# Zhen-Dong/CoDeNet

Hardware: AMD Instinct MI355X
Metric: images/sec CoDeNet1x 512x512 ctdet inference (deform hot path: deconv_layers; whole network in `e2e`) (higher is better)
Workload: dtype f32+i8 (W4A8: fp32 scale / gather, int8-MFMA pointwise on 8-bit activation and 4-bit weight codes, i32 sums); 1 GPU; CoDeNet1x config-c 512x512 W4A8, batch 64 per GPU, 3 deform stages (scale 1x1 -> QuantAct -> bilinear-gather depthwise 3x3 -> QuantAct -> pointwise 1x1 + folded BN -> ReLU -> QuantAct range; output channels-last at stage resolution for the native heads), running QuantAct ranges (reference-faithful), fused per-stage schedule, HIP-graph replay; preset=cfg3, global_batch=64

## Files before the change

### codenet_amd/_native.py

```python
import ctypes
import os
import subprocess

_HERE = os.path.dirname(os.path.abspath(__file__))
SO_PATH = os.path.join(_HERE, "lib", "libcodenet_dcn.so")
CSRC = os.path.join(_HERE, "csrc")

CDN_F32, CDN_F64, CDN_F16 = 0, 1, 2
_lib = None

_vp, _i, _i64, _f, _d = ctypes.c_void_p, ctypes.c_int, ctypes.c_int64, ctypes.c_float, ctypes.c_double

_SIGNATURES = {
    "cdn_abi_version": (ctypes.c_int, []),
    "cdn_last_error": (ctypes.c_char_p, []),
    "cdn_deform_conv_forward": (_i, [_vp] * 4 + [_i] + [_i64] * 5 + [_i] * 10 + [_vp]),
    "cdn_deform_conv_forward_scratch_bytes": (ctypes.c_size_t, [_i64] * 5 + [_i] * 10),
    "cdn_deform_conv_forward_scratch": (_i, [_vp] * 4 + [_i] + [_i64] * 5 + [_i] * 10 + [_vp, ctypes.c_size_t, _vp]),
    "cdn_deform_conv_backward_input": (_i, [_vp] * 6 + [_i] + [_i64] * 5 + [_i] * 10 + [_vp]),
    "cdn_deform_conv_backward_input_scratch_bytes": (ctypes.c_size_t, [_i64] * 5 + [_i] * 10),
    "cdn_deform_conv_backward_input_scratch_min_bytes": (ctypes.c_size_t, [_i64] * 5 + [_i] * 10),
    "cdn_deform_conv_backward_input_scratch": (_i, [_vp] * 6 + [_i] + [_i64] * 5 + [_i] * 10 + [_vp, ctypes.c_size_t, _vp]),
    "cdn_deform_conv_backward_parameters": (_i, [_vp] * 4 + [_i] + [_i64] * 5 + [_i] * 10 + [_f, _vp]),
    "cdn_modulated_deform_conv_forward": (_i, [_vp] * 6 + [_i] + [_i64] * 5 + [_i] * 11 + [_vp]),
    "cdn_modulated_deform_conv_backward": (_i, [_vp] * 11 + [_i] + [_i64] * 5 + [_i] * 11 + [_vp]),
    "cdn_codenet_scale_forward": (_i, [_vp] * 4 + [_i64] * 4 + [_f, _f, _vp]),
    "cdn_codenet_dw_forward": (_i, [_vp] * 4 + [_i64] * 4 + [_vp]),
    "cdn_codenet_dw_backward_supported": (_i, [_i64, _i64]),
    "cdn_codenet_pointwise_wgrad_workspace_bytes": (ctypes.c_size_t, [_i64] * 4),
    "cdn_codenet_pointwise_wgrad": (_i, [_vp] * 4 + [_i64] * 4 + [_vp, ctypes.c_size_t, _vp]),
    "cdn_codenet_scale_backward": (_i, [_vp] * 5 + [_i64] * 4 + [_vp]),
    "cdn_codenet_scale_range_partials": (_i64, [_i64] * 3),
    "cdn_codenet_scale_forward_range": (_i, [_vp] * 4 + [_i64] * 4 + [_f, _f, _vp, _vp]),
    "cdn_codenet_dw_range_partials": (_i64, [_i64] * 4),
    "cdn_codenet_dw_forward_range": (_i, [_vp] * 4 + [_i64] * 4 + [_vp, _vp]),
    "cdn_codenet_pointwise_range_partials": (_i64, [_i64] * 3),
    "cdn_codenet_pointwise_forward_range": (_i, [_vp] * 7 + [_i64] * 4 + [_i, _vp, _vp]),
    "cdn_quantact_forward_partials": (_i, [_vp, _vp, _i64, _vp, _vp, _vp, _vp, _i64, _i, _d, _i, _vp, _vp]),
    "cdn_codenet_pointwise_wgrad_q": (_i, [_vp] * 5 + [_i64] * 4 + [_vp, ctypes.c_size_t, _vp]),
    "cdn_codenet_pointwise_wgrad_q_f32": (_i, [_vp] * 5 + [_i64] * 4 + [_vp, ctypes.c_size_t, _vp]),
    "cdn_quantact_relu_up2_forward_partials": (
        _i, [_vp, _vp] + [_i64] * 3 + [_vp] * 4 + [_i64, _i, _d, _i, _vp]),
    "cdn_codenet_scale_backward_masked": (_i, [_vp] * 3 + [_f, _f] + [_vp] * 3 + [_i64] * 4 + [_vp]),
    "cdn_codenet_weight_prep_backward": (_i, [_vp] * 7 + [_i64, _i64] + [_vp] * 5),
    "cdn_codenet_weight_prep": (_i, [_vp, _i64, _i64] + [_vp] * 4 + [_i] + [_vp] * 3),
    "cdn_codenet_weight_prep_multi": (_i, [_i] + [_vp] * 14),
    "cdn_codenet_weight_prep_ranked": (_i, [_vp, _i64, _i64] + [_vp] * 4 + [_i, _i, _i, _f] + [_vp] * 3),
    "cdn_codenet_stage_supported": (_i, [_i64] * 4 + [_i, _i]),
    "cdn_codenet_stage_fused_supported": (_i, [_i64] * 4 + [_i, _i]),
    "cdn_codenet_stage_chain_parts": (_i, [_i64] * 5),
    "cdn_codenet_heads_pointwise_supported": (_i, [_i64, _i64, _i]),
    "cdn_codenet_heads_pointwise_forward": (_i, [_vp, _vp, _i64, _i64, _i] + [_vp] * 5 + [_i] + [_vp] * 3 + [_i, _d, _i]
                                            + [_vp, ctypes.c_size_t, _vp, _vp, _i64, _vp]),
    "cdn_codenet_stage_fused_forward_chain": (_i, [_vp, _i, _i, _vp] + [_i64] * 5 + [_vp, _vp, _f, _f] + [_vp] * 5
                                              + [_i, _vp, ctypes.c_size_t, _vp, _vp, _i, _vp, _vp, _vp]),
    "cdn_codenet_stage_fused_intermediates": (_i, [_i64] * 4 + [_i, _i, _i, _vp, _vp]),
    "cdn_codenet_wcodes_kb_columns": (_i64, [_i64, _i64]),
    "cdn_codenet_pointwise_i8_supported": (_i, [_i64] * 4),
    "cdn_quantact_arrive_words": (_i, []),
    "cdn_codenet_scale_forward_update": (_i, [_vp] * 4 + [_i64] * 4 + [_f, _f] + [_vp] * 4 + [_i, _d, _vp, _vp]),
    "cdn_codenet_dw_forward_update_supported": (_i, [_i64] * 4 + [_i]),
    "cdn_codenet_dw_forward_update": (_i, [_vp] * 4 + [_i64] * 4 + [_i] + [_vp] * 4 + [_i, _d, _vp, _vp]),
    "cdn_codenet_pointwise_i8_forward_update": (_i, [_vp] * 5 + [_i64] * 4 + [_vp, ctypes.c_size_t, _i] + [_vp] * 4
                                                + [_i, _d, _vp]),
    "cdn_quantact_apply": (_i, [_vp, _vp, _i64, _vp, _vp]),
    "cdn_quantact_relu_apply": (_i, [_vp, _vp, _i64, _i64, _i64, _i, _vp, _vp]),
    "cdn_codenet_pointwise_dgrad_q4_supported": (_i, [_i64] * 4),
    "cdn_codenet_pointwise_dgrad_q4": (_i, [_vp] * 3 + [_i64] * 4 + [_vp]),
    "cdn_codenet_pointwise_i8_workspace_bytes": (ctypes.c_size_t, [_i64] * 4),
    "cdn_codenet_pointwise_i8_range_partials": (_i64, [_i64] * 4),
    "cdn_codenet_pointwise_i8_forward_range": (_i, [_vp] * 5 + [_i64] * 4 + [_vp, _vp, ctypes.c_size_t, _vp]),
    "cdn_codenet_wcodes_kb_offset": (_i64, [_i64, _i64]),
    "cdn_codenet_maxpool3x3s2_q8_forward": (_i, [_vp] + [_i64] * 6 + [_vp, _vp]),
    "cdn_codenet_dwpw_q8_supported": (_i, [_i64] * 3 + [_i, _i64]),
    "cdn_codenet_dwpw_q8_forward": (
        _i, [_vp, _vp] + [_i64] * 4 + [_i, _i64, _vp, _vp, _i, _vp, _i64] + [_vp] * 4 + [_i, _i64] + [_vp] * 5),
    "cdn_codenet_dw_backward": (_i, [_vp] * 7 + [_i64] * 4 + [_vp]),
    "cdn_codenet_dw_backward_workspace_bytes": (ctypes.c_size_t, [_i64] * 4 + [_i]),
    "cdn_codenet_dw_backward_r": (_i, [_vp] * 7 + [_i64] * 4 + [_vp, _vp]),
    "cdn_codenet_dw_up2_backward_r": (_i, [_vp] * 7 + [_i64] * 4 + [_vp, _vp]),
    "cdn_codenet_pointwise_forward": (_i, [_vp] * 6 + [_i64] * 4 + [_i, _vp]),
    "cdn_quantact_state_bytes": (ctypes.c_size_t, []),
    "cdn_kth_values_workspace_bytes": (ctypes.c_size_t, []),
    "cdn_kth_values": (_i, [_vp, _i64, _i64, _i64, _vp, _vp, _vp, ctypes.c_size_t, _vp]),
    "cdn_quantact_forward": (_i, [_vp] * 3 + [_i64] + [_vp] * 5 + [_i, _d, _i, _vp]),
    "cdn_quantact_relu_up2_forward": (_i, [_vp, _vp] + [_i64] * 3 + [_vp] * 3 + [_i, _d, _i, _vp]),
    "cdn_up2_relu_backward": (_i, [_vp] * 3 + [_i64] * 3 + [_vp]),
    "cdn_quantact_relu_forward": (_i, [_vp, _vp, _i64] + [_vp] * 4 + [_i64, _i, _d, _i, _vp]),
    "cdn_relu_backward": (_i, [_vp] * 3 + [_i64, _vp]),
    "cdn_codenet_pwdw_s2_supported": (_i, [_i64] * 5),
    "cdn_codenet_pwdw_s2_forward": (
        _i, [_vp, _vp] + [_i64] * 5 + [_vp] * 8 + [_i64, _vp, _vp, _i64] + [_vp] * 3 + [_i, _d, _i, _vp,
                                                                                    ctypes.c_size_t, _vp, _vp]),
    "cdn_codenet_pwdw_s2_apply": (
        _i, [_vp, _vp] + [_i64] * 5 + [_vp] * 8 + [_i64, _vp, _vp, _i64] + [_vp] * 3 + [_i, _d, _i, _vp,
                                                                                    ctypes.c_size_t, _vp, _vp]),
    "cdn_codenet_dw_up2_supported": (_i, [_i64] * 4),
    "cdn_codenet_dw_up2_range_partials": (_i64, [_i64] * 4),
    "cdn_codenet_dw_up2_forward": (_i, [_vp] * 4 + [_i64] * 4 + [_vp, _vp]),
    "cdn_codenet_dw_up2_backward": (_i, [_vp] * 7 + [_i64] * 4 + [_vp]),
    "cdn_codenet_stage_workspace_bytes": (ctypes.c_size_t, [_i64] * 4 + [_i]),
    "cdn_codenet_stage_fused_forward": (
        _i, [_vp, _i, _i, _vp] + [_i64] * 5 + [_vp, _vp, _f, _f] + [_vp] * 8 + [_i] + [_vp] * 9
        + [_i, _d, _i, _vp, ctypes.c_size_t, _vp, _vp]),
    "cdn_quantact_commit_range": (_i, [_vp, _vp, _vp, _vp, _i, _d, _i, _vp]),
    "cdn_quantact_frozen_params": (_i, [_i, _vp, _vp, _vp, _i, _vp]),
    "cdn_quantact_frozen_params_clear": (_i, [_i, _vp, _vp, _vp, _i, _vp, ctypes.c_size_t, _vp]),
    "cdn_codenet_stage_frozen_workspace_bytes": (ctypes.c_size_t, [_i64] * 4 + [_i]),
    "cdn_codenet_stage_frozen_forward": (
        _i, [_vp, _i, _i, _vp] + [_i64] * 5 + [_vp, _vp, _f, _f] + [_vp] * 5 + [_i] + [_vp] * 4
# ... 161 lines not shown
```

### codenet_amd/csrc/codenet_pointwise.hip

```cpp
#include "cdn_common.h"

#include <algorithm>
#include <type_traits>

#ifdef CDN_STAMPS
__device__ unsigned long long cdn_pw_stamps[2048 * 8];
#define CDN_STAMPR(R, I)                                                                              \
  do {                                                                                                \
    static_assert((R) == 2, "the pointwise kernels stamp region 2");                                  \
    if (threadIdx.x == 0)                                                                             \
      cdn_pw_stamps[((blockIdx.y * gridDim.x + blockIdx.x) & 2047) * 8 + (I)] = __builtin_amdgcn_s_memrealtime(); \
  } while (0)
int cdn::read_pointwise_stamps(unsigned long long *host_dst) {
  return (int)hipMemcpyFromSymbol(host_dst, HIP_SYMBOL(cdn_pw_stamps), sizeof(unsigned long long) * 2048 * 8);
}
int cdn::clear_pointwise_stamps() {
  void *p = nullptr;
  if (hipGetSymbolAddress(&p, HIP_SYMBOL(cdn_pw_stamps)) != hipSuccess) return 1;
  return (int)hipMemset(p, 0, sizeof(unsigned long long) * 2048 * 8);
}
#else
#define CDN_STAMPR(R, I) do { } while (0)
#endif

// ... 676 lines not shown
          if (relu) v = cdn::relu_keep_nan(v);
          if (R) R[m * ldo + oc] = v;
          mn = fminf(mn, v);
          mx = fmaxf(mx, v);
          has_nan |= (v != v);
        }
      }
  }
  CDN_STAMPR(2, 3);
  if (qu.tracks())
    cdn::block_minmax_finish(cdn::nan_lo(mn, has_nan), cdn::nan_hi(mx, has_nan), pidx, npart, qu,
                             reinterpret_cast<float *>(&A0[0][0]));
  CDN_STAMPR(2, 4);
}

template <int BM, int BN, int WGM, bool FAST>
__global__ void __launch_bounds__(256)
pwi8_kernel(const float *__restrict__ A, const unsigned *__restrict__ aq,
            const signed char *__restrict__ Wq, const float *__restrict__ wscale,
            const int *__restrict__ wsum, const float *__restrict__ Wp,
            const float *__restrict__ bias, float *__restrict__ R,
            cdn::QUpdate qu, long M, int C, int Cpad, int Co, int relu, int lda,
            int ldo, const int *__restrict__ omap, int Cw) {
  pwi8_body<BM, BN, WGM, FAST>(A, aq, Wq, wscale, wsum, Wp, bias, R, qu, M, C, Cpad, Co, relu, lda, ldo, omap, Cw,
                               (long)blockIdx.x * BM, blockIdx.y * BN, blockIdx.y * gridDim.x + blockIdx.x,
                               gridDim.x * gridDim.y);
}

struct QUpdateN {
  cdn::QUpdate q[4];
};
template <int NH>
__global__ void __launch_bounds__(256)
pwi8h_kernel(const float *__restrict__ A, const unsigned *__restrict__ aq, const signed char *__restrict__ Wq,
             const float *__restrict__ wscale, const int *__restrict__ wsum, const float *__restrict__ Wp,
             const float *__restrict__ bias, float *__restrict__ R, QUpdateN qus, long M, int C, int Cpad,
             int relu, int lda, const int *__restrict__ omap, long head_stride) {
  const int ntm = (int)((M + 63) / 64), grp = 8 * NH, b = blockIdx.x, full = (ntm / 8) * grp;
  int mt, head;
  if (b < full) {
    const int lid = b % grp;
    head = lid >> 3;
    mt = (b - lid) / NH + (lid & 7);
  } else {
    const int q = b - full, rem = ntm - (full / NH);
    head = q / rem;
    mt = full / NH + q % rem;
  }
  pwi8_body<64, 64, 2, true>(A, aq, Wq, wscale, wsum, Wp, bias, R + (long)head * head_stride, qus.q[head],
                             M, C, Cpad, 64 * NH, relu, lda, 64, omap, C, (long)mt * 64, head * 64, mt, ntm);
}


template <int TN, int RR>
__device__ __forceinline__ void pwi8s_body(const float *__restrict__ A, const signed char *__restrict__ Wkb,
                                           const float *__restrict__ wscale, const int *__restrict__ wsum,
                                           const float *__restrict__ bias, float *__restrict__ R,
                                           const cdn::QUpdate &qu, long M, int K, int Co, int relu, int lda, int ldo,
                                           const int *__restrict__ omap, int ncg, long m0, int cb, float qs, float qz,
                                           char *lds) {
  constexpr int kRing = RR * 4096;
  __builtin_amdgcn_s_waitcnt(0x0F70);
  const int tid = threadIdx.x, lane = tid & 63;
  const int w = __builtin_amdgcn_readfirstlane(tid >> 6);
  const int i = lane & 31, h = lane >> 5;
  const int Cot = 32 * TN * ncg;
  const int ioff = (int)qz + (2048 - 128) - 0x4B400000;
  const int pairs = K >> 6;
  const int nit = 2 * ((pairs >> 2) + (w < (pairs & 3) ? 1 : 0));
  const int win0 = 2 * (w * (pairs >> 2) + min(w, pairs & 3)), kbase = 32 * win0;
  const float *abase = A + m0 * lda + kbase;
  unsigned aoff[4];
  {
    const int dr = lane >> 3, dc = lane & 7;
    const long rmax = M - 1 - m0;
#pragma unroll
    for (int u = 0; u < 4; ++u) {
      const int row = 8 * u + dr;
      const int rl = (int)(row < rmax ? row : rmax);
      aoff[u] = (unsigned)rl * (unsigned)lda * 4u + (unsigned)((dc ^ ((row >> 1) & 7)) * 16);
    }
  }
  const unsigned ring = cdn::lds_addr_uniform(lds) + (unsigned)w * kRing;
  auto issue = [&](int t) {
    const unsigned dst = ring + (unsigned)(t % RR) * 4096;
#pragma unroll
    for (int u = 0; u < 4; ++u) cdn::glds16(abase, aoff[u] + (unsigned)t * 128u, dst + u * 1024);
  };
  const unsigned long long wb = (unsigned long long)(Wkb + ((long)win0 * Cot + cb) * 32);
  const unsigned wlo = __builtin_amdgcn_readfirstlane((unsigned)wb), whi = __builtin_amdgcn_readfirstlane((unsigned)(wb >> 32));
  const unsigned long long wbu = ((unsigned long long)whi << 32) | wlo;
  const unsigned bo0 = (unsigned)(i * 32 + 16 * h), wstep = (unsigned)Cot * 32u;
  i32x4 bA[TN], bB[TN];
  auto loadB = [&](i32x4 (&b)[TN], int t) {
    static_assert(TN <= 4, "one offset register: the tiles of a window within the 13-bit immediate");
    const unsigned v0 = bo0 + (unsigned)t * wstep;
#pragma unroll
    for (int j = 0; j < TN; ++j)
      asm volatile("global_load_dwordx4 %0, %1, %2 offset:%3" : "=v"(b[j]) : "v"(v0), "s"(wbu), "n"(1024 * j) : "memory");
  };
  auto release = [&](i32x4 (&b)[TN]) {
    if constexpr (TN == 4)
      asm volatile("" : "+v"(b[0]), "+v"(b[1]), "+v"(b[2]), "+v"(b[3 % TN]));
    else
      asm volatile("" : "+v"(b[0]), "+v"(b[1]));
  };
  auto ucode = [&](float v) -> unsigned {
#pragma clang fp contract(off)
    const float y_p = qs * v;
    const float y = (y_p - qz) + 12582912.0f;
    int u = (int)__float_as_uint(y) + ioff;
    u = min(max(u, 8), 4087);
    return (unsigned)u;
  };
  i32x16 acc[TN];
#pragma unroll
  for (int j = 0; j < TN; ++j) acc[j] = (i32x16){0};
  const char *wring = lds + w * kRing;
  const int frow = i * 128, fsw = (i >> 1) & 7;
  CDN_STAMPR(2, 1);
#pragma unroll
  for (int t = 0; t < RR - 2; ++t) issue(t);
  loadB(bA, 0);
  issue(RR - 2);
  auto step = [&](int t, i32x4 (&bcur)[TN], i32x4 (&bnxt)[TN], auto more_b, auto more_a, auto prev_a) {
    constexpr int MB = decltype(more_b)::value, MA = decltype(more_a)::value, PA = decltype(prev_a)::value;
    if constexpr (MB) loadB(bnxt, t + 1);
    if constexpr (MA) issue(t + RR - 1);
    asm volatile("s_waitcnt vmcnt(%0)" ::"n"(TN * MB + 4 * MA + 4 * PA) : "memory");
    release(bcur);
    const char *slot = wring + (t % RR) * 4096;
    i32x4 a0, a1;
#pragma unroll
    for (int q = 0; q < 4; ++q) {
      const float4 v = *reinterpret_cast<const float4 *>(slot + frow + ((4 * h + q) ^ fsw) * 16);
      const unsigned u0 = ucode(v.x), u1 = ucode(v.y), u2 = ucode(v.z), u3 = ucode(v.w);
      const unsigned p01 = u0 | (u1 << 16), p23 = u2 | (u3 << 16);
      a0[q] = (int)(__builtin_amdgcn_perm(p23, p01, 0x06040200u) & 0x0F0F0F0Fu);
      a1[q] = (int)(__builtin_amdgcn_perm(p23 >> 4, p01 >> 4, 0x06040200u) ^ 0x80808080u);
    }
#pragma unroll
    for (int j = 0; j < TN; ++j) acc[j] = __builtin_amdgcn_mfma_i32_32x32x32_i8(a0, bcur[j], acc[j], 0, 0, 0);
#pragma unroll
    for (int j = 0; j < TN; ++j) {
      i32x4 s16;
#pragma unroll
      for (int e = 0; e < 4; ++e) s16[e] = (int)(((unsigned)bcur[j][e] << 4) & 0xF0F0F0F0u);
      acc[j] = __builtin_amdgcn_mfma_i32_32x32x32_i8(a1, s16, acc[j], 0, 0, 0);
    }
  };
  static_assert(RR == 3, "the peeled tail is written for a ring of three windows");
  {
    const std::true_type y;
    const std::false_type n;
    int t = 0;
    for (; t + 2 < nit; t += 2) {
      step(t, bA, bB, y, y, y);
      step(t + 1, bB, bA, y, y, y);
    }
    step(t, bA, bB, y, n, y);
    step(t + 1, bB, bA, n, n, n);
  }
  CDN_STAMPR(2, 2);
  float mn = INFINITY, mx = -INFINITY;
  bool has_nan = false;
  {
    int *P = reinterpret_cast<int *>(lds);
    constexpr int PLD = 36;
    const int col = tid & 63, r0 = (tid >> 6) * 8;
    for (int j0 = 0; j0 < TN; j0 += 2) {
      __syncthreads();
#pragma unroll
      for (int jj = 0; jj < 2; ++jj)
#pragma unroll
        for (int g = 0; g < 4; ++g) {
          const i32x16 &c = acc[j0 + jj];
          *reinterpret_cast<i32x4 *>(&P[((w * 64) + jj * 32 + i) * PLD + 8 * g + 4 * h]) =
              (i32x4){c[4 * g], c[4 * g + 1], c[4 * g + 2], c[4 * g + 3]};
        }
      __syncthreads();
      const int co = cb + j0 * 32 + col;
      if (co < Co) {
        const float bsv = bias ? bias[co] : 0.0f;
        const float rinv = __fdiv_rn(1.0f, __fmul_rn(qs, wscale[co]));
        const int t128 = 128 * wsum[co], oc = omap ? omap[co] : co;
        i32x4 s[2];
#pragma unroll
        for (int hh = 0; hh < 2; ++hh) {
          const i32x4 p0 = *reinterpret_cast<const i32x4 *>(&P[(0 * 64 + col) * PLD + r0 + 4 * hh]);
          const i32x4 p1 = *reinterpret_cast<const i32x4 *>(&P[(1 * 64 + col) * PLD + r0 + 4 * hh]);
          const i32x4 p2 = *reinterpret_cast<const i32x4 *>(&P[(2 * 64 + col) * PLD + r0 + 4 * hh]);
          const i32x4 p3 = *reinterpret_cast<const i32x4 *>(&P[(3 * 64 + col) * PLD + r0 + 4 * hh]);
          s[hh] = (p0 + p1) + (p2 + p3);
        }
#pragma unroll
        for (int rr = 0; rr < 8; ++rr) {
          const int row = r0 + rr;
          if (m0 + row < M) {
            float v = fmaf((float)(s[rr >> 2][rr & 3] + t128), rinv, bsv);
            if (relu) v = cdn::relu_keep_nan(v);
            if (R) R[(m0 + row) * ldo + oc] = v;
            mn = fminf(mn, v);
            mx = fmaxf(mx, v);
            has_nan |= (v != v);
          }
        }
      }
    }
  }
  CDN_STAMPR(2, 3);
  if (qu.tracks()) {
    __syncthreads();
    cdn::block_minmax_finish(cdn::nan_lo(mn, has_nan), cdn::nan_hi(mx, has_nan), blockIdx.x, gridDim.x, qu,
                             reinterpret_cast<float *>(lds));
  }
  CDN_STAMPR(2, 4);
}

template <int TN, int RR>
__global__ void __launch_bounds__(256)
pwi8s_kernel(const float *__restrict__ A, const unsigned *__restrict__ aq, const signed char *__restrict__ Wkb,
             const float *__restrict__ wscale, const int *__restrict__ wsum, const float *__restrict__ Wp,
             const float *__restrict__ bias, float *__restrict__ R, cdn::QUpdate qu, long M, int K,
             int Co, int relu, int lda, int ldo, const int *__restrict__ omap, int Cw, int ncg) {
  extern __shared__ float4 p8_lds[];
  char *lds = reinterpret_cast<char *>(p8_lds);
  CDN_STAMPR(2, 0);
  int rb = blockIdx.x, cg = 0;
  if (ncg == 2) {
    const int nrb8 = (int)((gridDim.x >> 1) & ~7u), b = blockIdx.x;
    if (b < 2 * nrb8) { rb = ((b >> 4) << 3) | (b & 7); cg = (b >> 3) & 1; }
    else { rb = nrb8 + ((b - 2 * nrb8) >> 1); cg = b & 1; }
  }
  const long m0 = (long)rb * 32;
  const int cb = cg * 32 * TN;
  const float qs = reinterpret_cast<const float *>(aq)[2];
  const float qz = reinterpret_cast<const float *>(aq)[3];
  if (aq[6] == 0) {
    pwi8s_body<TN, RR>(A, Wkb, wscale, wsum, bias, R, qu, M, K, Co, relu, lda, ldo, omap, ncg, m0, cb, qs, qz, lds);
  } else {
    float *fl = reinterpret_cast<float *>(lds);
    const int cend = min(Co, cb + 32 * TN);
    pwi8_wide_path<32, 128, 1>(A, Wp, bias, R, qu, M, Cw, cend, relu, lda, ldo, omap, qs, qz, fl, fl + 32 * 17,
                               fl + (32 + 128) * 17, m0, cb, (32 * TN + 127) / 128, (int)blockIdx.x, (int)gridDim.x);
  }
}
using bf16x8 = __attribute__((ext_vector_type(8))) __bf16;
constexpr int kB3LD = 80;

template <int BM, int BN, int WGM>
__global__ void __launch_bounds__(256)
pwb3_kernel(const float *__restrict__ A, const unsigned *__restrict__ aq,
            const signed char *__restrict__ Wq, const float *__restrict__ wscale,
            const float *__restrict__ bias, float *__restrict__ R, cdn::QUpdate qu,
            long M, int C, int Cpad, int Co, int relu, int lda, int ldo,
            const unsigned char *__restrict__ agen, const int *__restrict__ omap) {
  constexpr int WGN = 4 / WGM;
  constexpr int TM = BM / (WGM * 32), TN = BN / (WGN * 32);
  constexpr int AI = BM * 8 / 256;
  constexpr int BI = (BN * 2 + 255) / 256;
  __shared__ float2 qt[kMixedMaxC];
  __shared__ __attribute__((aligned(16))) unsigned char Ah[BM * kB3LD];
  __shared__ __attribute__((aligned(16))) unsigned char Am[BM * kB3LD];
  __shared__ __attribute__((aligned(16))) unsigned char Al[BM * kB3LD];
  __shared__ __attribute__((aligned(16))) unsigned char Bs[BN * kB3LD];
  const long m0 = (long)blockIdx.x * BM;
  const int n0 = blockIdx.y * BN;
  const int tid = threadIdx.x, lane = tid & 63, wave = tid >> 6;
  const int wm = (wave / WGN) * TM * 32, wn = (wave % WGN) * TN * 32;
  const bool has_q = aq != nullptr;
  const bool mixed = agen != nullptr;
  float qs = 1.f, qz = 0.f;
  if (has_q && !mixed) {
// ... 431 lines not shown
    for (int j = 0; j < TN; ++j)
#pragma unroll
      for (int r = 0; r < 16; ++r) {
        const long m = mb0 + (r & 3) + 8 * (r >> 2) + 4 * (lane >> 5);
        if (m < M && oc[j] >= 0) {
          float v = fmaf(acc[j][r], rinv[j], bsv[j]);
          if (relu) v = cdn::relu_keep_nan(v);
          R[m * ldo + oc[j]] = v;
          mn = fminf(mn, v);
          mx = fmaxf(mx, v);
          has_nan |= (v != v);
        }
      }
  }
  CDN_STAMPR(2, 3);
  if (qu.tracks())
    cdn::block_minmax_finish(cdn::nan_lo(mn, has_nan), cdn::nan_hi(mx, has_nan), blockIdx.y * gridDim.x + blockIdx.x,
                             gridDim.x * gridDim.y, qu, reinterpret_cast<float *>(smem));
  CDN_STAMPR(2, 4);
}

}

#ifndef CDN_PWS_MAX_TILES
#define CDN_PWS_MAX_TILES (cdn::kCUs)
#endif
static bool pws_applies(long M, int64_t K, int64_t Co, int64_t lda, const float *a, const float *w) {
  if (K < 32 || (K & 31) || (lda & 3) || ((reinterpret_cast<uintptr_t>(a) | reinterpret_cast<uintptr_t>(w)) & 15))
    return false;
  const long tiles = cdn::ceil_div(M, Co > 64 ? 64 : 128) * cdn::ceil_div(Co, Co > 64 ? 128 : 64);
  return tiles <= (long)CDN_PWS_MAX_TILES && cdn::ceil_div(M, 32) * cdn::ceil_div(Co, 32) <= (1L << 20);
}

static int pws_choice(long M, int64_t C, int64_t Co) {
  const long want = 4L * cdn::kCUs, mt32 = cdn::ceil_div(M, 32);
  const long w21 = mt32 * cdn::ceil_div(Co, 64), w11 = mt32 * cdn::ceil_div(Co, 32);
  const bool can_split = (C & 127) == 0;
  if (w21 >= want || (!can_split && Co > 32)) return 21;
  if (w11 >= want || !can_split) return 11;
  if (4 * w21 >= want) return 24;
  return 14;
}

static int64_t wcodes_kb_columns(int64_t Kpad, int64_t Co) {
#if defined(CDN_NO_PWI8S)
  return 0;
#endif
  if (Kpad < 512 || (Kpad & 63) || Co > 256 || Co < 1) return 0;
  return Co <= 64 ? 64 : Co <= 128 ? 128 : 256;
}
static bool pwi8s_applies(long M, int64_t Kt, int Cpad, int64_t Co, bool pw_fast, const signed char *w_kb) {
  return w_kb != nullptr && pw_fast && Kt == Cpad && wcodes_kb_columns(Kt, Co) != 0 && M >= 1 &&
         2 * cdn::ceil_div(M, 32) <= (long)kMaxGrid;
}
extern "C" int64_t cdn_codenet_wcodes_kb_columns(int64_t C, int64_t Co) {
  return C > 0 ? wcodes_kb_columns((C + 63) / 64 * 64, Co) : 0;
}
extern "C" int64_t cdn_codenet_wcodes_kb_offset(int64_t C, int64_t Co) {
  return C > 0 && Co > 0 ? (Co * ((C + 63) / 64 * 64) + 255) / 256 * 256 : 0;
}

int cdn::pointwise_chain_parts(long M, int64_t C, int64_t Co) {
  if (!pws_applies(M, C, Co, C, nullptr, nullptr)) return 0;
  return (int)cdn::ceil_div(Co, 32 * (pws_choice(M, C, Co) / 10));
}

int cdn::launch_pointwise(const cdn::PwCall &p) {
  const long M = p.M;
  const int64_t C = p.C, Co = p.Co, lda = p.lda ? p.lda : C, ldo = p.ldo ? p.ldo : Co;
  hipStream_t st = p.st;
  const int pw_bn = Co > 64 ? 128 : 64;
  const int pw_bm = (Co > 64 && cdn::ceil_div(M, 128) * cdn::ceil_div(Co, 128) <= cdn::kCUs) ? 64 : 128;
  const int n_wg_r = (int)(cdn::ceil_div(M, pw_bm) * cdn::ceil_div(Co, pw_bn));
  CDN_REQUIRE(n_wg_r <= kMaxGrid, CDN_ERR_UNSUPPORTED, "too many pointwise workgroups");
  const int64_t Kt = p.a_padded ? lda : C;
  const bool pw_fast = (Kt % 32) == 0 && (lda & 3) == 0 && (reinterpret_cast<uintptr_t>(p.a) & 15) == 0;
#define CDN_PW1(BM_, BN_, WGM_, AQ_, FAST_)                                                      \
  pw3_kernel<BM_, BN_, WGM_, AQ_, FAST_><<<(unsigned)std::min<long>(                             \
      cdn::ceil_div(M, BM_) * cdn::ceil_div(Co, BN_), only_if_wide ? 2L * cdn::kCUs : (1L << 30)), 256, 0, st>>>( \
      p.a, p.a_state, p.w, p.bias, p.ep_scale, p.ep_shift, p.out, p.qu, M, (int)C, (int)Co, p.relu, only_if_wide, \
      (int)lda, (int)ldo)
#define CDN_PW(BM_, BN_, WGM_, AQ_)                                       \
  do {                                                                    \
    if (pw_fast) CDN_PW1(BM_, BN_, WGM_, AQ_, true);                      \
    else CDN_PW1(BM_, BN_, WGM_, AQ_, false);                             \
  } while (0)
  const bool use_i8 = p.w_codes != nullptr && p.a_state != nullptr && p.ep_scale == nullptr && p.a_gen == nullptr;
  const bool use_b3 = p.w_codes != nullptr && p.ep_scale == nullptr && p.w_scale != nullptr &&
                      (p.a_gen != nullptr || p.a_state == nullptr);
  CDN_REQUIRE(p.a_gen == nullptr || (use_b3 && p.a_state != nullptr && C <= kMixedMaxC), CDN_ERR_UNSUPPORTED,
              "a mixed-generation input needs the states, 4-bit weight codes and C <= %d", kMixedMaxC);
  CDN_REQUIRE(p.out_map == nullptr || use_i8 || use_b3, CDN_ERR_UNSUPPORTED,
              "an output channel map needs the 4-bit weight codes");
  const int only_if_wide = 0;
  if (use_i8) {
    CDN_REQUIRE(p.w_scale && p.w_colsum, CDN_ERR_ARG, "int8 pointwise needs scale and colsum");
    CDN_REQUIRE((reinterpret_cast<uintptr_t>(p.w_codes) & 15) == 0, CDN_ERR_ARG,
                "w_pw_codes must be 16-byte aligned");
    const int Cpad = (int)((C + 63) / 64 * 64);
    CDN_REQUIRE(!p.a_padded || lda == Cpad, CDN_ERR_ARG, "a padded A has round_up(C, 64) floats per row");
    cdn::ProfScope ps(cdn::kProfPointwise, p.ptag, st);
#define CDN_PWI(BM_, BN_, WGM_)                                                                            \
  do {                                                                                                     \
    dim3 g((unsigned)cdn::ceil_div(M, BM_), (unsigned)cdn::ceil_div(Co, BN_));                             \
    auto kern = pw_fast ? pwi8_kernel<BM_, BN_, WGM_, true> : pwi8_kernel<BM_, BN_, WGM_, false>;          \
    kern<<<g, 256, 0, st>>>(p.a, p.a_state, p.w_codes, p.w_scale, p.w_colsum, p.w, p.bias, p.out, p.qu, M, \
                            (int)Kt, Cpad, (int)Co, p.relu, (int)lda, (int)ldo, p.out_map, (int)C);        \
  } while (0)
    if (pwi8s_applies(M, Kt, Cpad, Co, pw_fast, p.w_kb)) {
      const long nrb = cdn::ceil_div(M, 32);
      const int ncg = Co > 128 ? 2 : 1;
      const unsigned grid = (unsigned)(nrb * ncg);
      constexpr int kLds = 4 * 3 * 4096;
      auto kern = Co <= 64 ? pwi8s_kernel<2, 3> : pwi8s_kernel<4, 3>;
      kern<<<grid, 256, kLds, st>>>(p.a, p.a_state, p.w_kb, p.w_scale, p.w_colsum, p.w, p.bias, p.out, p.qu, M, (int)Kt,
                                    (int)Co, p.relu, (int)lda, (int)ldo, p.out_map, (int)C, ncg);
      return cdn::check_launch("codenet int8 pointwise (streaming)");
    }
#if !defined(CDN_NO_PWI32)
    if (pw_bn == 128 && cdn::ceil_div(M, 64) * cdn::ceil_div(Co, 128) <= cdn::kCUs && Kt >= 1024) CDN_PWI(32, 128, 1);
    else
#endif
#if !defined(CDN_PWI_NO_32ROWS)
    if (pw_bn == 128 && Kt < 256) CDN_PWI(32, 128, 1);
    else
#endif
    if (pw_bn == 128) CDN_PWI(64, 128, 2);
#if !defined(CDN_PWI_NO_64X64)
    else if (M >= 65536) CDN_PWI(64, 64, 2);
#endif
    else CDN_PWI(128, 64, 4);
#undef CDN_PWI
  } else if (use_b3) {
    CDN_REQUIRE((reinterpret_cast<uintptr_t>(p.w_codes) & 15) == 0, CDN_ERR_ARG,
                "w_pw_codes must be 16-byte aligned");
    const int Cpad = (int)((C + 63) / 64 * 64);
    cdn::ProfScope ps(cdn::kProfPointwise, p.ptag, st);
#define CDN_PWB(BM_, BN_, WGM_)                                                                           \
  do {                                                                                                    \
    dim3 g((unsigned)cdn::ceil_div(M, BM_), (unsigned)cdn::ceil_div(Co, BN_));                            \
    pwb3_kernel<BM_, BN_, WGM_><<<g, 256, 0, st>>>(p.a, p.a_state, p.w_codes, p.w_scale, p.bias, p.out, p.qu, M, \
                                                   (int)C, Cpad, (int)Co, p.relu, (int)lda, (int)ldo, p.a_gen,   \
                                                   p.out_map);                                            \
  } while (0)
    int tn = Co > 64 ? 4 : 2;
    const int Kp = (int)((C + 31) / 32 * 32);
#if !defined(CDN_PWD3_NO_TN2_SMALLM)
    if (tn == 4 && (size_t)32 * 4 * (Kp * 2 + 16) + (size_t)Kp * 16 > 80 * 1024 &&
        cdn::ceil_div(M, 256) * cdn::ceil_div(Co, 128) < cdn::kCUs)
      tn = 2;
#endif
    const size_t lds_d3 = (size_t)32 * tn * (Kp * 2 + 16) + (size_t)Kp * 16;
    const long nblk_d3 = cdn::ceil_div(M, 128) * cdn::ceil_div(Co, 32 * tn);
    if ((C & 3) == 0 && (lda & 3) == 0 && (reinterpret_cast<uintptr_t>(p.a) & 15) == 0 &&
        lds_d3 <= 150 * 1024 && nblk_d3 <= kMaxGrid) {
      const unsigned ny = (unsigned)cdn::ceil_div(Co, 32 * tn);
      const long per_cu = std::min<long>(tn == 2 ? 3 : 2, (long)(160 * 1024 / (lds_d3 + 512)));
      const long gx = std::max<long>(1, std::min<long>(cdn::ceil_div(M, 128), per_cu * cdn::kCUs / ny));
      dim3 g((unsigned)gx, ny);
      auto kern = tn == 4 ? pwd3_kernel<4> : pwd3_kernel<2>;
      (void)hipFuncSetAttribute((const void *)kern, hipFuncAttributeMaxDynamicSharedMemorySize, (int)lds_d3);
#if defined(CDN_PWD3_256)
      const int d3_threads = 256;
#else
      const int d3_threads = (per_cu == 1 && cdn::ceil_div(M, 256) * ny >= cdn::kCUs) ? 512 : 256;
#endif
      const long gx2 = std::max<long>(1, std::min<long>(cdn::ceil_div(M, d3_threads / 2), per_cu * cdn::kCUs / ny));
// ... 154 lines not shown
```

### include/codenet_dcn.h

```cpp
#ifndef CODENET_DCN_H_
#define CODENET_DCN_H_

#include <stddef.h>
#include <stdint.h>

#ifdef __cplusplus
extern "C" {
#endif

#define CDN_ABI_VERSION 1

enum cdn_dtype { CDN_F32 = 0, CDN_F64 = 1, CDN_F16 = 2 };

enum cdn_status {
  CDN_OK = 0,
  CDN_ERR_ARG = -1,
  CDN_ERR_SHAPE = -2,
  CDN_ERR_DTYPE = -3,
  CDN_ERR_HIP = -4,
  CDN_ERR_UNSUPPORTED = -5,
  CDN_ERR_WORKSPACE = -6
};

int cdn_abi_version(void);
// ... 144 lines not shown
int64_t cdn_codenet_dw_up2_range_partials(int64_t N, int64_t C, int64_t H, int64_t W);
int cdn_codenet_dw_up2_forward(const float *x_stored, const float *s_stored, const float *w_dw, float *d, int64_t N,
                               int64_t C, int64_t H, int64_t W, float *partials, void *stream);
int cdn_codenet_dw_up2_backward(const float *x_stored, const float *s_stored, const float *w_dw, const float *grad_d,
                                float *grad_x, float *grad_s, float *grad_w, int64_t N, int64_t C, int64_t H, int64_t W,
                                void *stream);
int cdn_codenet_dw_backward_supported(int64_t H, int64_t W);
int cdn_codenet_dw_backward(const float *x, const float *s, const float *w_dw,
                            const float *grad_d, float *grad_x, float *grad_s, float *grad_w,
                            int64_t N, int64_t C, int64_t H, int64_t W, void *stream);
size_t cdn_codenet_dw_backward_workspace_bytes(int64_t N, int64_t C, int64_t H, int64_t W, int up2);
int cdn_codenet_dw_backward_r(const float *x, const float *s, const float *w_dw, const float *grad_d, float *grad_x,
                              float *grad_s, float *grad_w, int64_t N, int64_t C, int64_t H, int64_t W,
                              float *workspace, void *stream);
int cdn_codenet_dw_up2_backward_r(const float *x_stored, const float *s_stored, const float *w_dw, const float *grad_d,
                                  float *grad_x, float *grad_s, float *grad_w, int64_t N, int64_t C, int64_t H,
                                  int64_t W, float *workspace, void *stream);

int cdn_codenet_pointwise_forward(const float *d, const float *w_pw, const float *bias,
                                  const float *ep_scale, const float *ep_shift, float *y,
                                  int64_t N, int64_t C, int64_t Co, int64_t HW, int relu,
                                  void *stream);

size_t cdn_quantact_state_bytes(void);

size_t cdn_kth_values_workspace_bytes(void);
int cdn_kth_values(const float *x, int64_t numel, int64_t k_lo, int64_t k_hi, float *out_lo, float *out_hi,
                   void *workspace, size_t workspace_bytes, void *stream);
int cdn_quantact_forward(const float *x, float *out, int16_t *codes, int64_t numel, float *x_min,
                         float *x_max, void *state, const float *batch_min,
                         const float *batch_max, int bits, double momentum, int running,
                         void *stream);
int cdn_quantact_relu_up2_forward(const float *y, float *out, int64_t planes, int64_t H, int64_t W, float *x_min,
                                  float *x_max, void *state, int bits, double momentum, int running, void *stream);
int cdn_up2_relu_backward(const float *grad_out, const float *y, float *grad_y, int64_t planes, int64_t H, int64_t W,
                          void *stream);
int cdn_quantact_relu_forward(const float *y, float *out, int64_t numel, float *x_min, float *x_max, void *state,
                              const float *partials, int64_t n_partials, int bits, double momentum, int running,
                              void *stream);
int cdn_relu_backward(const float *grad_out, const float *y, float *grad_y, int64_t numel, void *stream);

size_t cdn_codenet_stage_workspace_bytes(int64_t N, int64_t C, int64_t H, int64_t W, int x_up);
int cdn_codenet_stage_supported(int64_t N, int64_t C, int64_t H, int64_t W, int x_nhwc, int x_up);
int cdn_codenet_stage_fused_intermediates(int64_t N, int64_t C, int64_t H, int64_t W, int x_nhwc, int x_up,
                                          int int8_pointwise, int64_t *d_offset_bytes, int64_t *d_row_floats);
int cdn_codenet_stage_fused_supported(int64_t N, int64_t C, int64_t H, int64_t W, int x_nhwc, int x_up);
#define CDN_X_GATHER_PER_ITEM 0x100
#define CDN_X_GATHER_PERSISTENT 0x200
#define CDN_X_GATHER_MASK 0x300
#define CDN_X_ACT_PERCENTILE 0x400
#define CDN_X_WCODES_KB 0x800
int64_t cdn_codenet_wcodes_kb_columns(int64_t C, int64_t Co);
int64_t cdn_codenet_wcodes_kb_offset(int64_t C, int64_t Co);
#define CDN_X_DEFER_RANGE 0x1000
#define CDN_X_PHASE_SCALE 0x2000
#define CDN_X_PHASE_GATHER 0x4000
#define CDN_X_PHASE_POINTWISE 0x8000
#define CDN_X_PHASE_MASK 0xE000
int cdn_quantact_commit_range(float *x_min, float *x_max, void *state, const float *range, int bits, double momentum,
                              int running, void *stream);
int cdn_codenet_stage_fused_forward(
    const float *x, int x_nhwc, int x_up, const void *x_qstate, int64_t N, int64_t C, int64_t Co,
    int64_t H, int64_t W, const float *w_scale, const float *b_scale, float lo, float hi,
    const float *w_dw, const float *w_pw, const signed char *w_pw_codes, const float *w_pw_scale,
    const int *w_pw_colsum, const float *bias_pw, const float *ep_scale, const float *ep_shift,
    int relu, float *s_min, float *s_max, void *s_state, float *d_min,
    float *d_max, void *d_state, float *r_min, float *r_max, void *r_state, int bits,
    double momentum, int running, void *workspace, size_t workspace_bytes, float *r_out,
    void *stream);

int cdn_quantact_frozen_params(int n, float *const *x_min, float *const *x_max, void *const *state, int bits,
                               void *stream);
int cdn_quantact_frozen_params_clear(int n, float *const *x_min, float *const *x_max, void *const *state, int bits,
                                     void *clear, size_t clear_bytes, void *stream);
size_t cdn_codenet_stage_frozen_workspace_bytes(int64_t N, int64_t C, int64_t H, int64_t W, int x_up);
int cdn_codenet_stage_frozen_forward(
    const void *x, int x_kind, int x_up, const void *x_state, int64_t N, int64_t C, int64_t Co, int64_t H, int64_t W,
    const float *w_scale, const float *b_scale, float lo, float hi, const float *w_dw,
    const signed char *w_pw_codes, const float *w_pw_scale, const int *w_pw_colsum, const float *bias_pw, int relu,
    const void *s_state, const void *d_state, const void *r_state, void *workspace, size_t workspace_bytes,
    signed char *r8_out, unsigned *overflow, void *stream);
int cdn_codenet_stage_frozen_chained_forward(
    const void *x, int x_kind, int x_up, const void *x_state, int64_t N, int64_t C, int64_t Co, int64_t H, int64_t W,
    const float *w_scale, const float *b_scale, float lo, float hi, const float *w_dw,
    const signed char *w_pw_codes, const float *w_pw_scale, const int *w_pw_colsum, const float *bias_pw, int relu,
    const void *s_state, const void *d_state, const void *r_state, void *workspace, size_t workspace_bytes,
    signed char *r8_out, unsigned *overflow, const int *s_sums_in, const float *w_scale_sw,
    const signed char *next_scale_codes, int *s_sums_out, void *stream);
int cdn_codenet_pointwise_q8_forward(const signed char *a, const void *a_state, int64_t M, int64_t C, int64_t Co,
                                     const signed char *w_codes, const float *w_scale, const int *w_colsum,
                                     const float *bias, int relu, const void *r_state, signed char *r8_out,
                                     float *r_out, unsigned *overflow, void *stream);
int cdn_codenet_pointwise_q8_strided_forward(
    const signed char *a, const void *a_state, int64_t M, int64_t C, int64_t Co, int64_t lda, int64_t ldo,
    const signed char *w_codes, const float *w_scale, const int *w_colsum, const float *bias, int relu,
    const int *out_map, const void *r_state, signed char *r8_out, float *r_out, unsigned *overflow, void *stream);
int cdn_codenet_stem_q8_forward(const float *img, int64_t N, int64_t H, int64_t W, int64_t Co, int stride,
                                const float *w, const float *bias, int relu, const void *r_state,
                                signed char *out8, int64_t ld_out, unsigned *overflow, void *stream);
int cdn_codenet_maxpool3x3s2_q8_forward(const signed char *a8, int64_t N, int64_t C, int64_t H, int64_t W, int64_t ld_in,
                                        int64_t ld_out, signed char *out8, void *stream);
int cdn_codenet_dw3x3_q8_forward(const signed char *a8, const void *a_state, int64_t N, int64_t C, int64_t H,
                                 int64_t W, int stride, int64_t ld_in, int64_t ld_out, const float *w,
                                 const float *bias, int relu, const void *r_state, signed char *out8,
                                 unsigned *overflow, void *stream);
int cdn_codenet_dwpw_q8_supported(int64_t C, int64_t H, int64_t W, int stride, int64_t Co);
// ... 284 lines not shown
```

Before: 250,200 images/sec.

## Shrink streaming int8 pointwise ring to two windows and pin four waves per EU

Cuts the per-wave LDS ring in the streaming int8 pointwise kernel from three windows to two, so LDS drops from 48KB to the 36KB partial-sum footprint. It also requests four waves per EU and keeps offsets in uniform or precomputed vector registers to hold register pressure down. The prefetch pipeline is rebuilt as a one-step look-ahead. The aim is more resident workgroups per CU, at the cost of less prefetch depth to hide global-to-LDS latency. An occupancy query entry point is added for inspection.

Result: faster. 253,700 images/sec, median of 6 (+1.4%).

```diff
diff --git a/codenet_amd/_native.py b/codenet_amd/_native.py
--- a/codenet_amd/_native.py
+++ b/codenet_amd/_native.py
@@ -56,6 +56,7 @@
                                               + [_i, _vp, ctypes.c_size_t, _vp, _vp, _i, _vp, _vp, _vp]),
     "cdn_codenet_stage_fused_intermediates": (_i, [_i64] * 4 + [_i, _i, _i, _vp, _vp]),
     "cdn_codenet_wcodes_kb_columns": (_i64, [_i64, _i64]),
+    "cdn_codenet_pwi8s_resident_workgroups": (_i, [_i64]),
     "cdn_codenet_pointwise_i8_supported": (_i, [_i64] * 4),
     "cdn_quantact_arrive_words": (_i, []),
     "cdn_codenet_scale_forward_update": (_i, [_vp] * 4 + [_i64] * 4 + [_f, _f] + [_vp] * 4 + [_i, _d, _vp, _vp]),
diff --git a/codenet_amd/csrc/codenet_pointwise.hip b/codenet_amd/csrc/codenet_pointwise.hip
--- a/codenet_amd/csrc/codenet_pointwise.hip
+++ b/codenet_amd/csrc/codenet_pointwise.hip
@@ -752,6 +752,7 @@
 }
 
 
+constexpr int kPwi8sLds = 4 * 64 * 36 * 4;
 template <int TN, int RR>
 __device__ __forceinline__ void pwi8s_body(const float *__restrict__ A, const signed char *__restrict__ Wkb,
                                            const float *__restrict__ wscale, const int *__restrict__ wsum,
@@ -765,7 +766,8 @@
   const int w = __builtin_amdgcn_readfirstlane(tid >> 6);
   const int i = lane & 31, h = lane >> 5;
   const int Cot = 32 * TN * ncg;
-  const int ioff = (int)qz + (2048 - 128) - 0x4B400000;
+  const int ioff = __builtin_amdgcn_readfirstlane((int)qz + (2048 - 128) - 0x4B400000);
+  const int umax = __builtin_amdgcn_readfirstlane(4087);
   const int pairs = K >> 6;
   const int nit = 2 * ((pairs >> 2) + (w < (pairs & 3) ? 1 : 0));
   const int win0 = 2 * (w * (pairs >> 2) + min(w, pairs & 3)), kbase = 32 * win0;
@@ -779,13 +781,14 @@
       const int row = 8 * u + dr;
       const int rl = (int)(row < rmax ? row : rmax);
       aoff[u] = (unsigned)rl * (unsigned)lda * 4u + (unsigned)((dc ^ ((row >> 1) & 7)) * 16);
+      asm volatile("" : "+v"(aoff[u]));
     }
   }
   const unsigned ring = cdn::lds_addr_uniform(lds) + (unsigned)w * kRing;
   auto issue = [&](int t) {
     const unsigned dst = ring + (unsigned)(t % RR) * 4096;
 #pragma unroll
-    for (int u = 0; u < 4; ++u) cdn::glds16(abase, aoff[u] + (unsigned)t * 128u, dst + u * 1024);
+    for (int u = 0; u < 4; ++u) cdn::glds16(abase + t * 32, aoff[u], dst + u * 1024);
   };
   const unsigned long long wb = (unsigned long long)(Wkb + ((long)win0 * Cot + cb) * 32);
   const unsigned wlo = __builtin_amdgcn_readfirstlane((unsigned)wb), whi = __builtin_amdgcn_readfirstlane((unsigned)(wb >> 32));
@@ -810,30 +813,36 @@
     const float y_p = qs * v;
     const float y = (y_p - qz) + 12582912.0f;
     int u = (int)__float_as_uint(y) + ioff;
-    u = min(max(u, 8), 4087);
+    u = min(max(u, 8), umax);
     return (unsigned)u;
   };
   i32x16 acc[TN];
 #pragma unroll
   for (int j = 0; j < TN; ++j) acc[j] = (i32x16){0};
   const char *wring = lds + w * kRing;
-  const int frow = i * 128, fsw = (i >> 1) & 7;
+  unsigned foff[4];
+#pragma unroll
+  for (int q = 0; q < 4; ++q) {
+    foff[q] = (unsigned)(i * 128 + ((4 * h + q) ^ ((i >> 1) & 7)) * 16);
+    asm volatile("" : "+v"(foff[q]));
+  }
+  static_assert(RR == 2, "prologue, look-ahead and the peeled step are written for a ring of two windows");
   CDN_STAMPR(2, 1);
-#pragma unroll
-  for (int t = 0; t < RR - 2; ++t) issue(t);
   loadB(bA, 0);
-  issue(RR - 2);
-  auto step = [&](int t, i32x4 (&bcur)[TN], i32x4 (&bnxt)[TN], auto more_b, auto more_a, auto prev_a) {
-    constexpr int MB = decltype(more_b)::value, MA = decltype(more_a)::value, PA = decltype(prev_a)::value;
-    if constexpr (MB) loadB(bnxt, t + 1);
-    if constexpr (MA) issue(t + RR - 1);
-    asm volatile("s_waitcnt vmcnt(%0)" ::"n"(TN * MB + 4 * MA + 4 * PA) : "memory");
+  issue(0);
+  auto step = [&](int t, i32x4 (&bcur)[TN], i32x4 (&bnxt)[TN], auto more) {
+    constexpr int MORE = decltype(more)::value;
+    if constexpr (MORE) {
+      loadB(bnxt, t + 1);
+      issue(t + 1);
+    }
+    asm volatile("s_waitcnt vmcnt(%0)" ::"n"((TN + 4) * MORE) : "memory");
     release(bcur);
     const char *slot = wring + (t % RR) * 4096;
     i32x4 a0, a1;
 #pragma unroll
     for (int q = 0; q < 4; ++q) {
-      const float4 v = *reinterpret_cast<const float4 *>(slot + frow + ((4 * h + q) ^ fsw) * 16);
+      const float4 v = *reinterpret_cast<const float4 *>(slot + foff[q]);
       const unsigned u0 = ucode(v.x), u1 = ucode(v.y), u2 = ucode(v.z), u3 = ucode(v.w);
       const unsigned p01 = u0 | (u1 << 16), p23 = u2 | (u3 << 16);
       a0[q] = (int)(__builtin_amdgcn_perm(p23, p01, 0x06040200u) & 0x0F0F0F0Fu);
@@ -849,24 +858,27 @@
       acc[j] = __builtin_amdgcn_mfma_i32_32x32x32_i8(a1, s16, acc[j], 0, 0, 0);
     }
   };
-  static_assert(RR == 3, "the peeled tail is written for a ring of three windows");
   {
     const std::true_type y;
     const std::false_type n;
     int t = 0;
     for (; t + 2 < nit; t += 2) {
-      step(t, bA, bB, y, y, y);
-      step(t + 1, bB, bA, y, y, y);
-    }
-    step(t, bA, bB, y, n, y);
-    step(t + 1, bB, bA, n, n, n);
+      step(t, bA, bB, y);
+      step(t + 1, bB, bA, y);
+    }
+    step(t, bA, bB, y);
+    step(t + 1, bB, bA, n);
   }
   CDN_STAMPR(2, 2);
   float mn = INFINITY, mx = -INFINITY;
   bool has_nan = false;
   {
+    int etid = tid;
+    asm volatile("" : "+v"(etid));
+    const int tid = etid, i = tid & 31, h = (tid >> 5) & 1, w = __builtin_amdgcn_readfirstlane(tid >> 6);
     int *P = reinterpret_cast<int *>(lds);
     constexpr int PLD = 36;
+    static_assert(4 * 64 * PLD * 4 == kPwi8sLds && 4 * kRing <= kPwi8sLds, "the partial sums alias the rings");
     const int col = tid & 63, r0 = (tid >> 6) * 8;
     for (int j0 = 0; j0 < TN; j0 += 2) {
       __syncthreads();
@@ -918,7 +930,7 @@
 }
 
 template <int TN, int RR>
-__global__ void __launch_bounds__(256)
+__global__ void __launch_bounds__(256) __attribute__((amdgpu_waves_per_eu(4, 4)))
 pwi8s_kernel(const float *__restrict__ A, const unsigned *__restrict__ aq, const signed char *__restrict__ Wkb,
              const float *__restrict__ wscale, const int *__restrict__ wsum, const float *__restrict__ Wp,
              const float *__restrict__ bias, float *__restrict__ R, cdn::QUpdate qu, long M, int K,
@@ -1456,6 +1468,14 @@
 static bool pwi8s_applies(long M, int64_t Kt, int Cpad, int64_t Co, bool pw_fast, const signed char *w_kb) {
   return w_kb != nullptr && pw_fast && Kt == Cpad && wcodes_kb_columns(Kt, Co) != 0 && M >= 1 &&
          2 * cdn::ceil_div(M, 32) <= (long)kMaxGrid;
+}
+using Pwi8sKernel = decltype(&pwi8s_kernel<4, 2>);
+static Pwi8sKernel pwi8s_choice(int64_t Co) { return Co <= 64 ? pwi8s_kernel<2, 2> : pwi8s_kernel<4, 2>; }
+extern "C" int cdn_codenet_pwi8s_resident_workgroups(int64_t Co) {
+  if (Co < 1 || Co > 256) return 0;
+  int n = 0;
+  const hipError_t e = hipOccupancyMaxActiveBlocksPerMultiprocessor(&n, (const void *)pwi8s_choice(Co), 256, kPwi8sLds);
+  return e == hipSuccess ? n : -(int)e;
 }
 extern "C" int64_t cdn_codenet_wcodes_kb_columns(int64_t C, int64_t Co) {
   return C > 0 ? wcodes_kb_columns((C + 63) / 64 * 64, Co) : 0;
@@ -1515,8 +1535,8 @@
       const long nrb = cdn::ceil_div(M, 32);
       const int ncg = Co > 128 ? 2 : 1;
       const unsigned grid = (unsigned)(nrb * ncg);
-      constexpr int kLds = 4 * 3 * 4096;
-      auto kern = Co <= 64 ? pwi8s_kernel<2, 3> : pwi8s_kernel<4, 3>;
+      auto kern = pwi8s_choice(Co);
+      constexpr int kLds = kPwi8sLds;
       kern<<<grid, 256, kLds, st>>>(p.a, p.a_state, p.w_kb, p.w_scale, p.w_colsum, p.w, p.bias, p.out, p.qu, M, (int)Kt,
                                     (int)Co, p.relu, (int)lda, (int)ldo, p.out_map, (int)C, ncg);
       return cdn::check_launch("codenet int8 pointwise (streaming)");
diff --git a/include/codenet_dcn.h b/include/codenet_dcn.h
--- a/include/codenet_dcn.h
+++ b/include/codenet_dcn.h
@@ -220,6 +220,7 @@
 #define CDN_X_WCODES_KB 0x800
 int64_t cdn_codenet_wcodes_kb_columns(int64_t C, int64_t Co);
 int64_t cdn_codenet_wcodes_kb_offset(int64_t C, int64_t Co);
+int cdn_codenet_pwi8s_resident_workgroups(int64_t Co);
 #define CDN_X_DEFER_RANGE 0x1000
 #define CDN_X_PHASE_SCALE 0x2000
 #define CDN_X_PHASE_GATHER 0x4000
```
